# tensorflow/compression

Hardware: AMD Instinct MI355X
Metric: Mpixels/s encode+decode round-trip (bit-exact) (higher is better)
Workload: dtype int32

## Files before the change

compression_amd/_lib.py:

```python
from __future__ import annotations

import ctypes as C
import os

_HERE = os.path.dirname(os.path.abspath(__file__))
LIB_PATH = os.path.join(_HERE, "libtfc_hip.so")

_vp = C.c_void_p
_i64 = C.c_int64
_int = C.c_int

SIGNATURES = {
    "tfc_abi_version": (_int, []),
    "tfc_last_error": (C.c_char_p, []),
    "tfc_profile_enable": (None, [_int]),
    "tfc_set_default_mode": (_int, [_int]),
    "tfc_get_default_mode": (_int, []),
    "tfc_set_chip_shared": (_int, [_int]),
    "tfc_image_to_unit": (_int, [_vp, _vp, _int, C.c_int64, _vp]),
    "tfc_unit_to_image": (_int, [_vp, _int, _vp, C.c_int64, _vp]),
    "tfc_index_prepare": (_int, [_vp, _int, _vp, C.c_int64, _int, _vp]),
    "tfc_build_tables": (_int, [_vp, C.c_int64, C.c_int64, _vp, _vp, C.c_int64, _int, _vp, _vp]),
    "tfc_build_tables_overflow": (_int, [_vp, C.c_int64, C.c_int64, _vp, _vp, C.c_int64, _int, _vp, _vp, _vp]),
    "tfc_deep_factorized_tails": (_int, [_vp, C.c_int64, C.c_int64, _int, _int, _vp, _int, _vp, _vp, _vp]),
    "tfc_pad2d": (_int, [_vp, _vp, _int, C.c_int64, C.c_int64, C.c_int64, C.c_int64, _int, _int, _int, _int, _int, _vp]),
    "tfc_cache_bytes": (_int, [C.POINTER(C.c_longlong)]),
    "tfc_cache_trim": (_int, [C.POINTER(C.c_longlong)]),
    "tfc_encoder_capacity": (_int, [_vp, C.POINTER(_i64)]),
    "tfc_profile_query": (_int, [C.c_char_p, C.POINTER(C.c_double), C.POINTER(_i64)]),
    "tfc_pipe_counters": (_int, [C.POINTER(_i64), C.POINTER(_i64)]),
    "tfc_set_pipe_format": (_int, [_int, _int]),
    "tfc_tables_create": (_int, [_vp, _int, _i64, _i64, _vp, C.POINTER(_vp)]),
    "tfc_tables_count": (_i64, [_vp]),
    "tfc_tables_destroy": (None, [_vp]),
    "tfc_encoder_create": (_int, [_vp, _i64, _vp, C.POINTER(_vp)]),
    "tfc_encoder_create_many": (_int, [_vp, _i64, _int, _vp, _vp]),
    "tfc_encoder_set_mode": (_int, [_vp, _int]),
    "tfc_encoder_set_deferred_errors": (_int, [_vp, _int]),
    "tfc_encoder_encode": (_int, [_vp, _vp, _vp, _i64, _vp]),
    "tfc_encoder_encode_many": (_int, [_int, _vp, _vp, _vp, _i64, _vp]),
    "tfc_encoder_encode_quantized": (_int, [_vp, _vp, _int, _vp, _vp, _i64, _i64, _vp]),
    "tfc_encoder_encode_quantized_indexed": (_int, [_vp, _vp, _int, _vp, _vp, _i64, _vp]),
    "tfc_encoder_encode_quantized_many": (_int, [_int, _vp, _vp, _int, _vp, _vp, _i64, _i64, _vp]),
    "tfc_decoder_decode_dequantized_many": (_int, [_int, _vp, _vp, _int, _vp, _vp, _i64, _i64, _vp]),
    "tfc_encoder_encode_quantized_indexed_many": (_int, [_int, _vp, _vp, _int, _vp, _vp, _i64, _vp]),
    "tfc_decoder_decode_dequantized_indexed_many": (_int, [_int, _vp, _vp, _vp, _int, _vp, _i64, _vp]),
    "tfc_encoder_finalize": (_int, [_vp, _vp, C.POINTER(_i64)]),
    "tfc_encoder_finalize_device": (_int, [_vp, _vp]),
    "tfc_encoder_finalize_device_many": (_int, [_int, _vp, _vp]),
    "tfc_encoder_status": (_int, [_vp, _vp, C.POINTER(_i64)]),
    "tfc_encoder_result": (_int, [_vp, C.POINTER(_vp), C.POINTER(_vp)]),
    "tfc_encoder_read": (_int, [_vp, _vp, _vp, _int, _vp]),
    "tfc_encoder_destroy": (None, [_vp]),
    "tfc_decoder_create": (_int, [_vp, _vp, _vp, _i64, _int, _vp, C.POINTER(_vp)]),
    "tfc_decoder_create_many": (_int, [_vp, _int, _vp, _vp, _vp]),
    "tfc_decoder_set_mode": (_int, [_vp, _int]),
    "tfc_decoder_decode": (_int, [_vp, _vp, _vp, _i64, _vp]),
    "tfc_decoder_decode_many": (_int, [_int, _vp, _vp, _vp, _i64, _vp]),
    "tfc_decoder_decode_dequantized": (_int, [_vp, _vp, _vp, _int, _vp, _vp, _i64, _i64, _vp]),
    "tfc_decoder_finalize": (_int, [_vp, _vp, _vp]),
    "tfc_decoder_finalize_device": (_int, [_vp, _vp, _vp]),
    "tfc_decoder_finalize_device_many": (_int, [_int, _vp, _vp, _vp]),
    "tfc_decoder_status": (_int, [_vp, _vp]),
    "tfc_decoder_destroy": (None, [_vp]),
    "tfc_range_encode": (_int, [_vp, _vp, _int, _vp, _vp, _int, _int, _int, _vp,
                                C.POINTER(_vp), C.POINTER(_i64)]),
    "tfc_range_decode": (_int, [_vp, _i64, _vp, _int, _vp, _vp, _int, _int, _int, _vp, _vp]),
    "tfc_unbounded_index_range_encode": (_int, [_vp, _vp, _i64, _vp, _i64, _i64, _vp, _vp, _int, _int, _int,
                                                _vp, C.POINTER(_vp), C.POINTER(_i64)]),
    "tfc_unbounded_index_range_decode": (_int, [_vp, _i64, _vp, _i64, _vp, _i64, _i64, _vp, _vp, _int, _int,
                                                _int, _vp, _vp]),
    "tfc_stochastic_round": (_int, [_vp, _int, _i64, C.c_float, _vp, _i64, _vp, _vp]),
    "tfc_free": (None, [_vp]),
    "tfc_run_length_workspace": (_i64, [_i64, _i64]),
    "tfc_run_length_encode_size": (_int, [_vp, _int, _i64, _i64, _int, _int, _int, _vp, _vp, C.POINTER(_i64), _vp]),
    "tfc_run_length_encode_write": (_int, [_vp, _int, _i64, _i64, _int, _int, _int, _vp, _vp, _vp, _vp]),
    "tfc_run_length_decode": (_int, [_vp, _vp, _vp, _i64, _i64, _int, _int, _int, _int, _vp, _vp, _vp]),
    "tfc_pmf_to_quantized_cdf": (_int, [_vp, _i64, _i64, _int, _vp, _vp]),
    "tfc_gdn_forward": (_int, [_vp, _vp, _int, _i64, _i64, _vp, _vp, _int, _int, _int, _int, _vp]),
    "tfc_gdn_params_create": (_int, [_vp, _vp, _i64, _int, _vp, C.POINTER(_vp)]),
    "tfc_gdn_params_destroy": (None, [_vp]),
    "tfc_gdn_forward_prepared": (_int, [_vp, _vp, _vp, _i64, _int, _int, _int, _int, _vp]),
    "tfc_gdn_forward_general": (_int, [_vp, _vp, _int, _i64, _i64, _vp, _vp, _int, _int, C.c_float, C.c_float, _vp]),
# ... 138 lines not shown
```

compression_amd/csrc/range_coder.hip:

```cpp
#include <hip/hip_bf16.h>
#include <hip/hip_fp16.h>
#include <hip/hip_runtime.h>

#include <algorithm>
#include <atomic>
#include <cstdlib>
#include <cstring>
#include <type_traits>
#include <memory>
#include <mutex>
#include <string>
#include <vector>

#include "../../include/tfc_hip.h"
#include "common.h"
#include "range_coder_device.h"
#include "range_tables.h"
#include "range_wave.h"

using namespace tfc;


namespace tfc {

// ... 1288 lines not shown
  if (n <= 0) return 0;
  bool batch = n <= kMaxFinalizeJobs;
  for (int k = 0; k < n; ++k) es[k]->touch(st);
  for (int k = 0; k < n && batch; ++k) {
    const tfc_encoder* e = es[k];
    if (e->finalized || e->family != kLanes || e->chunks.size() != 1 || e->streams != es[0]->streams ||
        e->streams == 0 || e->chunks[0].stride != es[0]->chunks[0].stride)
      batch = false;
  }
  if (!batch) {
    for (int k = 0; k < n; ++k)
      if (tfc_encoder_finalize_device(es[k], stream)) return 1;
    return 0;
  }
  const int64_t streams = es[0]->streams;
  FinalizeJobs f;
  f.streams = streams;
  f.n = n;
  const size_t cap = es[0]->chunks[0].data_bytes + 4 * static_cast<size_t>(streams) + 64;
  f.length_off = static_cast<long long>((sizeof(Tail) * streams + 15) & ~size_t{15});
  f.offsets_off = f.length_off + static_cast<long long>(sizeof(long long)) * streams;
  f.blob_off = (f.offsets_off + static_cast<long long>(sizeof(long long)) * (streams + 1) + 15) & ~15ll;
  f.job_bytes = (f.blob_off + static_cast<long long>(cap) + 255) & ~255ll;
  auto group = std::make_shared<DevBuf>();
  TFC_HIP(group->alloc(static_cast<size_t>(f.job_bytes) * n, st));
  f.base = group->as<uint8_t>();
  for (int k = 0; k < n; ++k) {
    EncChunk& c = es[k]->chunks[0];
    f.job[k].state = es[k]->state.as<uint4>();
    f.job[k].chunk = ChunkRef{c.data.as<uint8_t>(), c.off.as<long long>(), c.len_p, c.stride};
  }
  hipLaunchKernelGGL(enc_tail_many_kernel, dim3(static_cast<unsigned>(ceil_div(streams, 256)), static_cast<unsigned>(n)),
                     dim3(256), 0, st, f);
  hipLaunchKernelGGL(scan_lengths_many_kernel, dim3(static_cast<unsigned>(n)), dim3(1024), 0, st, f);
  hipLaunchKernelGGL(enc_pack_many_kernel,
                     dim3(static_cast<unsigned>(ceil_div(streams, kWavesPerBlock)), static_cast<unsigned>(n)),
                     dim3(kBlock), 0, st, f);
  TFC_HIP(hipGetLastError());
  for (int k = 0; k < n; ++k) {
    tfc_encoder* e = es[k];
    e->result_group = group;
    e->offsets.p = f.base + k * f.job_bytes + f.offsets_off;
    e->blob.p = f.base + k * f.job_bytes + f.blob_off;
    e->blob_capacity = static_cast<int64_t>(cap);
    e->chunks.clear();
    e->finalized = true;
  }
  return 0;
}

extern "C" int tfc_debug_pipe_clocks(unsigned long long* out8) {
  TFC_HIP(hipDeviceSynchronize());
  TFC_HIP(hipMemcpyFromSymbol(out8, HIP_SYMBOL(tfc::g_pipe_clock), 8 * sizeof(unsigned long long)));
  return 0;
}
extern "C" int tfc_debug_enc_clocks(unsigned long long* out4) {
  TFC_HIP(hipDeviceSynchronize());
  TFC_HIP(hipMemcpyFromSymbol(out4, HIP_SYMBOL(tfc::g_enc_clock), 4 * sizeof(unsigned long long)));
  return 0;
}

extern "C" int tfc_pipe_counters(int64_t* launches, int64_t* fallback_blocks) {
  if (launches) *launches = pipe_launches().load();
  if (fallback_blocks) {
    unsigned long long v = 0;
    TFC_HIP(hipDeviceSynchronize());
    TFC_HIP(hipMemcpyFromSymbol(&v, HIP_SYMBOL(tfc::g_pipe_fallback_blocks), sizeof(v)));
    *fallback_blocks = static_cast<int64_t>(v);
  }
  return 0;
}

extern "C" int tfc_set_pipe_format(int format, int waves_per_workgroup) {
  if (format < 0 || format > 2 || waves_per_workgroup < 0 || waves_per_workgroup > 8) {
    tfc::fail("tfc_set_pipe_format: format 0 ... 2, waves per workgroup 0 ... 8");
    return -1;
  }
  pipe_waves_value().store(waves_per_workgroup);
  return pipe_format_value().exchange(format);
}

extern "C" int tfc_encoder_set_mode(tfc_encoder* e, int mode) {
  if (mode != TFC_MODE_AUTO && mode != TFC_MODE_LATENCY && mode != TFC_MODE_THROUGHPUT)
    return fail("unknown mode %d", mode);
  if (e->family >= 0) return fail("the mode of a handle is fixed by its first coding call");
  e->mode = mode;
  return 0;
}

extern "C" int tfc_encoder_set_deferred_errors(tfc_encoder* e, int on) {
  e->deferred = on != 0;
  return 0;
}

extern "C" int tfc_encoder_encode(tfc_encoder* e, const int32_t* value, const int32_t* index,
                                  int64_t elems, void* stream) {
  const SymInt32 src{value};
  return encode_jobs(&e, 1, &src, &index, elems, static_cast<hipStream_t>(stream), "tfc_encoder_encode");
}

extern "C" int tfc_encoder_encode_many(int n, tfc_encoder* const* es, const int32_t* const* values,
                                       const int32_t* const* indexes, int64_t elems, void* stream) {
  if (n <= 0) return 0;
  std::vector<SymInt32> srcs(n);
  for (int k = 0; k < n; ++k) srcs[k] = SymInt32{values[k]};
  return encode_jobs(es, n, srcs.data(), indexes, elems, static_cast<hipStream_t>(stream), "tfc_encoder_encode_many");
// ... 720 lines not shown
```

compression_amd/csrc/range_lanes.h:

```cpp
#pragma once

namespace tfc {

__device__ unsigned long long g_pipe_fallback_blocks;
__device__ unsigned long long g_pipe_clock[8];
__device__ unsigned long long g_enc_clock[4];

struct LaneArgs {
  const uint32_t* image;
  int bytes;
  int ntab;
  int precision;
  unsigned int cap;
  int lds_image;
  int lds_wave;
  int defer;
  const unsigned int* guard;
};

__device__ inline unsigned int lds_u16(const unsigned char* lds, unsigned int off) {
  return *reinterpret_cast<const unsigned short*>(lds + off);
}

__device__ inline unsigned int scale16(unsigned int s1, unsigned int c) {
  unsigned int add = c;
  asm volatile("" : "+v"(add));
  return static_cast<unsigned int>((static_cast<unsigned long long>(s1) * c + add) >> 16);
}

constexpr int kLaneJobArgBytes = 3584;
template <typename Src>
struct EncLaneJob {
  Src src;
  const int32_t* index;
  uint4* state;
  uint8_t* chunk;
  unsigned int* chunk_len;
  unsigned long long* first_error;
  unsigned int* overflow_flag;
};
template <typename Src>
struct EncLaneJobs {
  int64_t streams, elems;
  int blocks_per_job, n;
  static constexpr int kMax = kLaneJobArgBytes / sizeof(EncLaneJob<Src>) < 64 ? kLaneJobArgBytes / sizeof(EncLaneJob<Src>) : 64;
  EncLaneJob<Src> job[kMax];
};
template <typename Dst>
struct DecLaneJob {
  Dst dst;
  const int32_t* index;
  const uint8_t* blob;
  const long long* off;
  uint4* state;
  unsigned long long* first_error;
};
template <typename Dst>
struct DecLaneJobs {
// ... 18 lines not shown
  lanes_u32x4 v = {lo.x, lo.y, hi.x, hi.y};
  reinterpret_cast<TFC_AS1 LanePacked<lanes_u32x4>*>((TFC_AS1 void*)p)->v = v;
}
template <typename T>
__device__ inline void lanes_gstore_elem(T* p, const T& v) {
  if (sizeof(T) == 2) {
    unsigned short bits;
    __builtin_memcpy(&bits, &v, 2);
    reinterpret_cast<TFC_AS1 LanePacked<unsigned short>*>((TFC_AS1 void*)p)->v = bits;
  } else {
    unsigned int bits;
    __builtin_memcpy(&bits, &v, 4);
    reinterpret_cast<TFC_AS1 LanePacked<unsigned int>*>((TFC_AS1 void*)p)->v = bits;
  }
}

__device__ inline void lanes_load_image(unsigned char* lds, const LaneArgs& a) {
  const uint4* src = reinterpret_cast<const uint4*>(a.image);
  uint4* dst = reinterpret_cast<uint4*>(lds);
  const int n = (a.bytes + 15) / 16, step = static_cast<int>(blockDim.x);
  int i = threadIdx.x;
  for (; i + 7 * step < n; i += 8 * step) {
    uint4 v[8];
#pragma unroll
    for (int u = 0; u < 8; ++u) v[u] = lanes_gload16(src + i + u * step);
#pragma unroll
    for (int u = 0; u < 8; ++u) dst[i + u * step] = v[u];
  }
  for (; i < n; i += step) dst[i] = src[i];
  __syncthreads();
}

__device__ inline void lanes_pin(unsigned int& a, unsigned int& b, unsigned int& c, unsigned int& d) {
  asm volatile("" : "+v"(a), "+v"(b), "+v"(c), "+v"(d));
}


template <int WORDS>
struct LaneWindow {
  unsigned char* lds;
  const unsigned char* g;
  unsigned int len;
  unsigned int base;
  unsigned int pbase;
  uint2 pend[WORDS];

  __device__ __noinline__ unsigned int tail_word(unsigned int q0) const {
    unsigned int word = 0u;
#pragma nounroll
    for (unsigned int k = 0; k < 4u; ++k)
      if (q0 + k < len) word |= static_cast<unsigned int>(lanes_gload8(g + q0 + k)) << (8u * k);
    return word;
  }
  __device__ void request(unsigned int pos) {
    pbase = pos;
    if (pos + 8u * WORDS <= len) {
#pragma unroll
      for (int w = 0; w < WORDS; w += 2) {
#if defined(TFC_PDEC_ABL) && (TFC_PDEC_ABL & 2)
        const uint4 v = w == 0 ? lanes_gload16(g + pos) : make_uint4(pend[0].x, pend[0].y, pend[1].x, pend[1].y);
#else
        const uint4 v = lanes_gload16(g + pos + 8u * w);
#endif
        pend[w] = make_uint2(v.x, v.y);
        pend[w + 1] = make_uint2(v.z, v.w);
      }
    } else {
#pragma unroll
      for (int w = 0; w < WORDS; ++w) {
        pend[w].x = tail_word(pos + 8u * w);
        pend[w].y = tail_word(pos + 8u * w + 4u);
      }
    }
  }
  __device__ void commit() {
#pragma unroll
    for (int w = 0; w < WORDS; ++w) reinterpret_cast<uint2*>(lds)[w] = pend[w];
    base = pbase;
  }
};

__host__ __device__ constexpr int lane_stride(int payload) {
  return ((payload + 7) & ~7) + ((((payload + 7) & ~7) % 16 == 0) ? 8 : 0);
}


constexpr unsigned int kEncDigitBytes = 32;

template <typename Raw>
struct EncWaveLds {
  static constexpr int kValueWords = 2 * kEncCadence * sizeof(Raw) / 8;
  static constexpr int kIndexWords = 2 * kEncCadence * 4 / 8;
  static constexpr int kDigitStride = lane_stride(kEncDigitBytes + 8);
  static constexpr int kValueStride = lane_stride(8 * kValueWords);
  static constexpr int kIndexStride = lane_stride(8 * kIndexWords);
  static constexpr int kDigits = 0;
  static constexpr int kValue = kDigits + 64 * kDigitStride;
  static constexpr int kIndex = kValue + 64 * kValueStride;
  static constexpr int kBytes = kIndex + 64 * kIndexStride;
};

#define TFC_LENC_A(VAL, R0, R1, LO, HI, NEXTROW, NP)                                        \
  NEXTROW                                                                                 \
  "v_and_b32 v171, 0x7fffffff, v" #R1 "\n\t"                                              \
  "v_cmp_ge_u32 " NP(VAL)                                                                 \
  "v_min_u32 v172, v" #VAL ", v171\n\t"                                                   \
  "v_lshl_add_u32 v172, v172, 1, v" #R0 "\n\t"                                            \
  "ds_read_u16 v" #LO ", v172 offset:2\n\t"                                               \
  "ds_read_u16 v" #HI ", v172 offset:4\n\t"
#define TFC_LENC_B(LO, LOH, HI, HIH, PRE)                                                 \
  PRE                                                                                     \
  "v_mad_u64_u32 v[160:161], s[52:53], v" #LO ", %[S], v[" #LO ":" #LOH "]\n\t"             \
  "v_mad_u64_u32 v[162:163], s[52:53], v" #HI ", %[S], v[" #HI ":" #HIH "]\n\t"             \
  "v_alignbit_b32 v160, v161, v160, 16\n\t"                                               \
  "v_alignbit_b32 v162, v163, v162, 16\n\t"                                               \
  "v_add_u32 v162, -1, v162\n\t"                                                          \
  "v_min_u32 v162, v162, %[S]\n\t"                                                        \
  "v_add_co_u32 v164, vcc, %[BASE], v160\n\t"                                             \
  "v_addc_co_u32 v167, vcc, 0, %[H], vcc\n\t"                                             \
  "v_sub_u32 v165, v162, v160\n\t"                                                        \
  "v_sub_u32 v173, v167, %[H]\n\t"                                                        \
  "v_cmp_gt_u32 vcc, %[K64K], v165\n\t"                                                   \
  "v_cndmask_b32 v174, 0, 1, vcc\n\t"                                                     \
  "v_perm_b32 v166, 0, v167, %[PERM]\n\t"                                                 \
  "ds_write_b16 %[NA], v166\n\t"                                                          \
  "v_or_b32 v168, v173, v174\n\t"                                                         \
  "v_and_b32 v168, v168, %[HAD]\n\t"                                                      \
  "v_lshl_add_u32 %[NA], v168, 1, %[NA]\n\t"                                              \
  "v_lshrrev_b32 v169, 16, v164\n\t"                                                      \
  "v_lshlrev_b32 v170, 16, v164\n\t"                                                      \
  "v_lshl_or_b32 v171, v165, 16, %[KFFFF]\n\t"                                            \
  "v_cndmask_b32 %[BASE], v164, v170, vcc\n\t"                                            \
// ... 872 lines not shown
```

compression_amd/csrc/range_pipe.h:

```cpp
#pragma once

#ifndef TFC_PIPE_TIMING
#define TFC_PIPE_TIMING 0
#endif

namespace tfc {

constexpr int kPipeTile = 256;
constexpr int kPipeEscMax = 32;
constexpr unsigned int kPipeBlock = 16;
constexpr unsigned int kPipeNoCall = 0x0001FFFFu;
constexpr unsigned int kPipeAggregate = 1u << 30;
constexpr unsigned int kPipePrefix = 2u << 30;
constexpr unsigned int kPipeRowsMask = (1u << 30) - 1u;

struct PipeEncArgs {
  const uint16_t* fast16;
  const int2* rows_fast;
  int ntab;
  int tab_entries;
  unsigned int* calls;
  unsigned int* status;
  unsigned int* done;
  unsigned int* fallback;
// ... 842 lines not shown
  if (M < 0) return bit ? -M : (M == -31 ? 32 : M - 1);
  return M - 1;
}

struct PipeDecArgs {
  unsigned short* raw;
  unsigned int* posrec;
  unsigned int* kend;
  uint4* state_out;
  const unsigned short* rowaddr;
  unsigned int* fallback;
  unsigned int* progress;
  unsigned int* tile_done;
  unsigned int* started;
  int rows;
  int groups_per_job;
  int groups;
  int concurrent;
  long long poll_ticks;
};
constexpr unsigned int kPipeFinal = 0x80000000u;
#ifndef TFC_PIPE_RELEASE
#define TFC_PIPE_RELEASE 64
#endif
constexpr unsigned int kPipeRelease = TFC_PIPE_RELEASE;
struct PipeDecJob { const uint8_t* blob; const long long* off; const uint4* state; };
struct PipeDecJobs {
  int64_t streams, elems;
  int blocks_per_job, n;
  PipeDecJob job[64];
};

struct PipeRowJobs {
  int64_t per_job;
  int ntab, n;
  struct { const int32_t* index; unsigned long long* first_error; } job[64];
};
__global__ void __launch_bounds__(256) dec_rows_kernel(const PipeRowJobs jobs, unsigned short* rowaddr) {
  const int k = blockIdx.y;
  const int32_t* index = jobs.job[k].index;
  unsigned short* out = rowaddr + static_cast<size_t>(k) * jobs.per_job;
  for (int64_t i = static_cast<int64_t>(blockIdx.x) * 1024 + threadIdx.x, e = min(jobs.per_job, (static_cast<int64_t>(blockIdx.x) + 1) * 1024);
       i < e; i += 256) {
    int t = tfc_gload(index + i);
    if (t < 0 || t >= jobs.ntab) {
      atomicMin(jobs.job[k].first_error, static_cast<unsigned long long>(i));
      t = 0;
    }
    out[i] = static_cast<unsigned short>(16 * t);
  }
}

struct PipeDecLds {
  static constexpr int kWords = 2 * kPipeBlock * 2 / 8 + 2;
  static constexpr int kStride = lane_stride(8 * kWords);
  static constexpr int kCodes = 0;
  static constexpr int kRows = kCodes + 64 * kStride;
  static constexpr int kBytes = kRows + 64 * kStride;
  static constexpr int kStage = kPipeBlock * 128;
};

#ifndef TFC_PDEC_ABL
#define TFC_PDEC_ABL 0
#endif
#if TFC_PDEC_ABL & 1
#define TFC_PDEC_STORE(KOFF)
#define TFC_PDEC_WAIT2 "s_waitcnt lgkmcnt(1)\n\t"
#else
#define TFC_PDEC_STORE(KOFF) "ds_write_b16 %[STG], v117 offset:" #KOFF "\n\t"
#define TFC_PDEC_WAIT2 "s_waitcnt lgkmcnt(2)\n\t"
#endif
#ifndef TFC_PDEC_PAD
#define TFC_PDEC_PAD 0
#endif
#define TFC_PDEC_PAD2 "v_mov_b32 v139, v139\n\tv_mov_b32 v139, v139\n\t"
#if TFC_PDEC_PAD == 1
#define TFC_PDEC_PAD_A TFC_PDEC_PAD2
#elif TFC_PDEC_PAD == 5
#define TFC_PDEC_PAD_A "s_waitcnt lgkmcnt(15)\n\ts_waitcnt lgkmcnt(15)\n\t"
#else
#define TFC_PDEC_PAD_A
#endif
#if TFC_PDEC_PAD == 2
#define TFC_PDEC_PAD_B TFC_PDEC_PAD2
#else
#define TFC_PDEC_PAD_B
#endif
#if TFC_PDEC_PAD == 3
#define TFC_PDEC_PAD_C TFC_PDEC_PAD2
#else
#define TFC_PDEC_PAD_C
#endif
#if TFC_PDEC_PAD == 4
#define TFC_PDEC_PAD_D TFC_PDEC_PAD2
#else
#define TFC_PDEC_PAD_D
#endif
#define TFC_PDEC_STEP(KOFF, MI, MO, AHEAD, NEXT, PWSTEP)                                    \
  "v_cvt_f32_u32 v111, %[S]\n\t"                                                          \
  "v_add_f32 v111, 1.0, v111\n\t"                                                         \
  "v_rcp_f32 v111, v111\n\t"                                                              \
  TFC_PDEC_PAD_A                                                                          \
  "v_cvt_f32_u32 v110, %[D]\n\t"                                                          \
  "v_fma_f32 v110, -v110, %[SCALE], -%[HSCALE]\n\t"                                       \
  "v_fma_f32 v110, v110, v111, -1.0\n\t"                                                  \
  "v_cvt_i32_f32 v110, v110\n\t"                                                          \
  "v_ashrrev_i32 v111, 6, v110\n\t"                                                       \
// ... 307 lines not shown
            if (D < A) sym = sym > 0u ? sym - 1u : 0u;
            else sym = sym + 1u < nsym ? sym + 1u : nsym - 1u;
            lo = lds_u16(lanes_lds, R.x + 2u * sym + 2u);
            hi = lds_u16(lanes_lds, R.x + 2u * sym + 4u);
            A = scale16(s1, lo);
            b = scale16(s1, hi) - 1u;
            b = hi == 0u ? s1 : b;
          }
        }
        D -= A;
        s1 = b - A;
        const bool ren = (s1 >> 16) == 0u;
        D = ren ? (D << 16) | dig : D;
        s1 = ren ? (s1 << 16) | 0xFFFFu : s1;
        cp += ren ? 2u : 0u;
        entry = pipe_raw_entry(sym, 0);
        M = ((R.y >> 15) & 1u) != 0u && sym == (R.y & 0x7FFFu) ? -1 : 0;
        }
      } else {
        const unsigned int half = scale16(s1, 32768u);
        const unsigned int bit = D >= half ? 1u : 0u;
        const unsigned int A = bit ? half : 0u;
        const unsigned int b = bit ? s1 : half - 1u;
        D -= A;
        s1 = b - A;
        const bool ren = (s1 >> 16) == 0u;
        D = ren ? (D << 16) | dig : D;
        s1 = ren ? (s1 << 16) | 0xFFFFu : s1;
        cp += ren ? 2u : 0u;
        entry = PAIRS ? 0x8001u + bit : pipe_raw_entry(bit, M);
        if (M < 0) {
          if (bit) M = -M;
          else M = M == -31 ? 32 : M - 1;
        } else {
          --M;
        }
      }
      if (M == 0) {
        ++pos;
        pw += INDEXED ? 2u : 16u;
        if (!INDEXED && pw == dir_end) pw = 0u;
        load_row();
      } else {
        R = bin;
      }
      if (to_stage) *reinterpret_cast<unsigned short*>(lanes_lds + stg + 128u * (row - k)) = static_cast<unsigned short>(entry);
      else raw[static_cast<size_t>(row) * 64 + lane] = static_cast<unsigned short>(entry);
    }
  };

#if TFC_PIPE_TIMING
  unsigned long long t_asm = 0ull, n_asm = 0ull, t_commit = 0ull, t_rest = 0ull;
#endif
  auto memory_phase = [&]() __attribute__((always_inline)) {
#if TFC_PIPE_TIMING
    const unsigned long long tm0 = clock64();
#endif
    const unsigned int cpos = cw.base + (cp - cw_off);
    cw.commit();
    cp = cw_off + (cpos - cw.base);
    if (INDEXED) {
      iw.commit();
      pw = iw_off + (2u * pos - iw.base);
    }
#if TFC_PIPE_TIMING
    asm volatile("s_waitcnt lgkmcnt(0)" ::: "memory");
    const unsigned long long tm1 = clock64();
    t_commit += tm1 - tm0;
#endif
    flush();
    if (k != 0u && (k / kPipeBlock) % kPipeRelease == 0u) {
      posrec[static_cast<size_t>(k / kPipeBlock) * 64] = pos + (M != 0 ? 1u : 0u);
      __builtin_amdgcn_fence(__ATOMIC_RELEASE, "agent");
      if (lane == 0u) __hip_atomic_store(&pa.progress[gi], k, __ATOMIC_RELAXED, __HIP_MEMORY_SCOPE_AGENT);
    }
    cw.request(cpos);
    if (INDEXED) iw.request(2u * pos);
    posrec[static_cast<size_t>(k / kPipeBlock) * 64] = pos + (M != 0 ? 1u : 0u);
#if TFC_PIPE_TIMING
    t_rest += clock64() - tm1;
#endif
  };
  auto fast_block = [&](unsigned int& flag) __attribute__((always_inline)) {
#define TFC_PDEC_OPERANDS                                                                                              \
        : [D] "+v"(D), [S] "+v"(s1), [CP] "+v"(cp), [M] "+v"(M), [PW] "+v"(pw), [FLAG] "+v"(flag),                    \
          [R0] "+v"(R.x), [R1] "+v"(R.y), [R2] "+v"(R.z), [R3] "+v"(R.w)                                              \
        : [STG] "v"(stg), [BINROW] "v"(bin_addr_v), [SCALE] "s"(scale), [HSCALE] "v"(hscale),        \
          [K64K] "s"(0x10000u), [KFFFF] "s"(0xFFFFu), [PERM] "s"(0x05040001u), [NSH] "s"(pair_nsh) \
        : "vcc", "memory", "s52", "s53", "s54", "s55", "s56", "s57", "s58", "s59", "v104", "v105", "v106", "v107", "v108", "v109", "v110", "v111", "v112", "v113", \
          "v114", "v115", "v116", "v117", "v118", "v119", "v122", "v123", "v124", "v125", "v126", "v127", "v128",      \
          "v129", "v130", "v131", "v132", "v133", "v134", "v135", "v136", "v137", "v138", "v139", "v140", "v141", "v142", "v143", "v144", "v145"
#if TFC_PIPE_TIMING
    const unsigned long long ta = clock64();
#endif
    if constexpr (INDEXED && PAIRS) asm volatile(TFC_PDEC_BLOCK(TFC_PDEC_STEP_PIX) TFC_PDEC_OPERANDS);
    else if constexpr (PAIRS) asm volatile(TFC_PDEC_BLOCK(TFC_PDEC_STEP_PCH) TFC_PDEC_OPERANDS);
    else if constexpr (INDEXED) asm volatile(TFC_PDEC_BLOCK(TFC_PDEC_STEP_IX) TFC_PDEC_OPERANDS);
    else asm volatile(TFC_PDEC_BLOCK(TFC_PDEC_STEP_CH) TFC_PDEC_OPERANDS);
#if TFC_PIPE_TIMING
    t_asm += clock64() - ta;
    ++n_asm;
#endif
  };
  auto fast_step = [&](unsigned int& flag, unsigned int slot) __attribute__((always_inline)) {
    const unsigned int stg_row = stg + 128u * slot;
    {
      const unsigned int stg = stg_row;
      if constexpr (INDEXED && PAIRS) asm volatile(TFC_PDEC_ONE(TFC_PDEC_STEP_PIX) TFC_PDEC_OPERANDS);
      else if constexpr (PAIRS) asm volatile(TFC_PDEC_ONE(TFC_PDEC_STEP_PCH) TFC_PDEC_OPERANDS);
      else if constexpr (INDEXED) asm volatile(TFC_PDEC_ONE(TFC_PDEC_STEP_IX) TFC_PDEC_OPERANDS);
      else asm volatile(TFC_PDEC_ONE(TFC_PDEC_STEP_CH) TFC_PDEC_OPERANDS);
    }
#undef TFC_PDEC_OPERANDS
  };
  bool gave_up = false;
  while (__any(pos < elems)) {
    if (lds0 == 0u && row_loaded && (INDEXED || static_cast<unsigned int>(la.ntab) >= kPipeBlock)) {
      while (__all(!live || (pos + kPipeBlock <= elems && M > -16)) && k + kPipeBlock <= static_cast<unsigned int>(pa.rows)) {
        memory_phase();
        const unsigned int D0 = D, s10 = s1, cp0 = cp, pw0 = pw;
        const int M0 = M;
        const uint4 R0 = R;
        unsigned int flag = 0u;
        fast_block(flag);
        if (__builtin_expect(__any(live && flag != 0u), 0)) {
          D = D0; s1 = s10; cp = cp0; pw = pw0; M = M0; R = R0;
#pragma nounroll
          for (unsigned int i = 0; i < kPipeBlock; ++i) {
            const unsigned int D1 = D, s11 = s1, cp1 = cp, pw1 = pw;
            const int M1 = M;
            const uint4 R1 = R;
            unsigned int f1 = 0u;
            if (live) fast_step(f1, i);
            if (__any(live && f1 != 0u)) {
              D = D1; s1 = s11; cp = cp1; pw = pw1; M = M1; R = R1;
              gstep(live, k + i, true);
            } else {
              pos += (pw - pw1) / (INDEXED ? 2u : 16u);
              if (!INDEXED) pw -= pw >= dir_end ? dir_end : 0u;
            }
          }
          staged = true;
          staged_k = k;
          k += kPipeBlock;
          continue;
        }
        pos += (pw - pw0) / (INDEXED ? 2u : 16u);
        if (!INDEXED) pw -= pw >= dir_end ? dir_end : 0u;
        staged = true;
        staged_k = k;
        k += kPipeBlock;
      }
      if (!__any(pos < elems)) break;
    }
    if (k + kPipeBlock > static_cast<unsigned int>(pa.rows)) {
      gave_up = true;
      break;
    }
    memory_phase();
    if (!row_loaded) {
      if (M == 0) load_row(); else R = bin;
      row_loaded = true;
    }
    const bool whole = pos + kPipeBlock <= elems;
    const bool blocks = __any(whole);
    if (blocks && __any(!whole && pos < elems && M != 0)) {
      if (pos < elems) {
#pragma unroll
        for (unsigned int i = 0; i < kPipeBlock; ++i) raw[static_cast<size_t>(k + i) * 64 + lane] = static_cast<unsigned short>(kPipeSkipRow);
      }
#pragma nounroll
      for (unsigned int i = 0; i < kPipeBlock; ++i) gstep(!whole && pos < elems && M != 0, k + i);
      k += kPipeBlock;
      continue;
    }
    const bool busy = blocks ? whole : pos < elems;
    const bool sitting = blocks && !whole && pos < elems;
    if (__builtin_expect(lds0 == 0u && blocks && !__any(busy && M <= -16), 1)) {
      if (__any(sitting)) {
        if (sitting) {
#pragma unroll
          for (unsigned int i = 0; i < kPipeBlock; ++i) *reinterpret_cast<unsigned short*>(lanes_lds + stg + 128u * i) = static_cast<unsigned short>(kPipeSkipRow);
        }
      }
      const unsigned int D0 = D, s10 = s1, cp0 = cp, pw0 = pw;
      const int M0 = M;
      const uint4 R0 = R;
      unsigned int flag = 0u;
      if (busy) {
        fast_block(flag);
      }
      if (__builtin_expect(!__any(flag != 0u), 1)) {
        if (busy) {
          pos += (pw - pw0) / (INDEXED ? 2u : 16u);
        }
        if (!INDEXED)
          while (__any(busy && pw >= dir_end)) pw -= pw >= dir_end ? dir_end : 0u;
        staged = true;
        staged_k = k;
        k += kPipeBlock;
        continue;
      }
      D = D0; s1 = s10; cp = cp0; pw = pw0; M = M0; R = R0;
    }
    if (sitting) {
#pragma unroll
      for (unsigned int i = 0; i < kPipeBlock; ++i) raw[static_cast<size_t>(k + i) * 64 + lane] = static_cast<unsigned short>(kPipeSkipRow);
    }
#pragma nounroll
    for (unsigned int i = 0; i < kPipeBlock; ++i) gstep(busy && pos < elems, k + i);
    k += kPipeBlock;
  }
  flush();
  posrec[static_cast<size_t>(k / kPipeBlock) * 64] = pos;
  if (gave_up) {
    if (lane == 0) {
      atomicOr(&pa.fallback[job], 1u);
      __hip_atomic_store(&pa.progress[gi], kPipeFinal, __ATOMIC_RELEASE, __HIP_MEMORY_SCOPE_AGENT);
    }
    return;
  }
  if (lane == 0) pa.kend[gi] = k;
  __builtin_amdgcn_fence(__ATOMIC_RELEASE, "agent");
  if (lane == 0) __hip_atomic_store(&pa.progress[gi], k | kPipeFinal, __ATOMIC_RELAXED, __HIP_MEMORY_SCOPE_AGENT);
  if (gi == 0 && lane == 0) {
    g_pipe_clock[2] = clock64() - clk0;
    g_pipe_clock[3] = wall_clock64() - wall0;
#if TFC_PIPE_TIMING
    g_pipe_clock[5] = t_asm | (t_commit << 32);
    g_pipe_clock[7] = n_asm | (static_cast<unsigned long long>(k) << 16) | (t_rest << 32);
#endif
  }
  if (live) {
    const unsigned int cpos = cw.base + (cp - cw_off);
    const unsigned char* srcp = J.blob + o0;
    unsigned int window = 0u;
    for (int i = -4; i < 0; ++i) {
      const long long q = static_cast<long long>(cpos) + i;
      window = (window << 8) | ((q >= 0 && q < static_cast<long long>(len)) ? srcp[q] : 0u);
    }
    pa.state_out[static_cast<size_t>(gi) * 64 + lane] = make_uint4(window - D, s1, window, cpos >> 1);
  }
}

constexpr int kParseRows = 128;
constexpr unsigned int kParseMargin = 96;

constexpr int kParseEscTables = 2048;

struct PipePairMap { const int* adjust; };
template <bool INDEXED, bool PAIRS, typename Dst>
__global__ void __launch_bounds__(256) dec_parse_kernel(const DecLaneJobs<Dst> jobs, const PipeDecArgs pa, const DecRow* dir, int ntab,
                                                        const PipePairMap pm) {
  constexpr int kPitch = 66;
  __shared__ unsigned short buf[kParseRows * kPitch];
  __shared__ unsigned int escsym[kParseEscTables];
  __shared__ unsigned int incomplete;
  const unsigned int tiles = static_cast<unsigned int>(pa.rows) / kParseRows + 1u;
  const unsigned int gi = blockIdx.x % static_cast<unsigned int>(pa.groups), kt = blockIdx.x / static_cast<unsigned int>(pa.groups);
  const unsigned int job = gi / static_cast<unsigned int>(pa.groups_per_job);
  const unsigned int wv = gi % static_cast<unsigned int>(pa.groups_per_job);
  const DecLaneJob<Dst>& J = jobs.job[job];
  const unsigned int tid = threadIdx.x, lane = tid & 63u;
  const unsigned int k0 = kt * kParseRows;
  unsigned int* const tile_done = pa.tile_done + static_cast<size_t>(gi) * tiles + kt;
  unsigned int kend;
  bool final = true;
  if (pa.concurrent) {
    const unsigned int need = k0 + kParseRows + kParseMargin;
    unsigned int* const abandon = pa.started + 1;
    unsigned int v = 0u;
    if (tid == 0u) {
      unsigned int seen = ~0u, go = 1u;
      long long t0 = 0;
      if (__hip_atomic_load(abandon, __ATOMIC_RELAXED, __HIP_MEMORY_SCOPE_AGENT) != 0u) go = 0u;
      while (go) {
        v = __hip_atomic_load(&pa.progress[gi], __ATOMIC_RELAXED, __HIP_MEMORY_SCOPE_AGENT);
        if ((v & kPipeFinal) || v >= need) break;
        const long long now = static_cast<long long>(wall_clock64());
        if (v != seen) { seen = v; t0 = now; }
// ... 115 lines not shown
```

include/tfc_hip.h:

```cpp
#ifndef TFC_HIP_H_
#define TFC_HIP_H_

#include <stdint.h>

#ifdef __cplusplus
extern "C" {
#endif

typedef struct tfc_tables tfc_tables;
typedef struct tfc_encoder tfc_encoder;
typedef struct tfc_decoder tfc_decoder;

#define TFC_ABI_VERSION 2
int tfc_abi_version(void);
const char* tfc_last_error(void);

void tfc_profile_enable(int on);
int tfc_profile_query(const char* kernel, double* total_ms, int64_t* launches);
int tfc_pipe_counters(int64_t* launches, int64_t* fallback_blocks);
int tfc_set_pipe_format(int format, int waves_per_workgroup);

#define TFC_MODE_AUTO 0
#define TFC_MODE_LATENCY 1
#define TFC_MODE_THROUGHPUT 2
int tfc_set_default_mode(int mode);
int tfc_get_default_mode(void);

int tfc_set_chip_shared(int shared);
int tfc_image_to_unit(const void* x, void* y, int dtype, int64_t n, void* stream);
int tfc_unit_to_image(const void* x, int dtype, void* y, int64_t n, void* stream);
int tfc_index_prepare(const void* indexes, int dtype, int32_t* out, int64_t n, int num_tables, void* stream);
int tfc_pad2d(const void* x, void* y, int elem_bytes, int64_t n, int64_t h, int64_t w, int64_t c, int top, int bottom,
              int left, int right, int reflect, void* stream);
int tfc_cache_bytes(long long* bytes);
int tfc_cache_trim(long long* released);


int tfc_tables_create(const int32_t* lookup, int rank, int64_t rows, int64_t cols,
                      void* stream, tfc_tables** out);
int64_t tfc_tables_count(const tfc_tables* t);
void tfc_tables_destroy(tfc_tables* t);


int tfc_encoder_create(const tfc_tables* tables, int64_t streams, void* stream,
                       tfc_encoder** out);

int tfc_encoder_create_many(const tfc_tables* tables, int64_t streams, int n, void* stream,
                            tfc_encoder** out);

int tfc_encoder_set_mode(tfc_encoder* e, int mode);
int tfc_encoder_set_deferred_errors(tfc_encoder* e, int on);

int tfc_encoder_encode(tfc_encoder* e, const int32_t* value, const int32_t* index,
                       int64_t elems, void* stream);

int tfc_encoder_encode_many(int n, tfc_encoder* const* e, const int32_t* const* value,
                            const int32_t* const* index, int64_t elems, void* stream);

int tfc_encoder_encode_quantized(tfc_encoder* e, const void* y, int dtype,
                                 const float* qoffset, const int32_t* cdf_offset,
                                 int64_t channels, int64_t elems, void* stream);

int tfc_encoder_encode_quantized_indexed(tfc_encoder* e, const void* y, int dtype,
                                         const int32_t* index, const int32_t* cdf_offset,
                                         int64_t elems, void* stream);

int tfc_encoder_encode_quantized_many(int n, tfc_encoder* const* e, const void* const* y, int dtype,
                                      const float* qoffset, const int32_t* cdf_offset,
                                      int64_t channels, int64_t elems, void* stream);
int tfc_encoder_encode_quantized_indexed_many(int n, tfc_encoder* const* e, const void* const* y, int dtype,
                                              const int32_t* const* index, const int32_t* cdf_offset,
                                              int64_t elems, void* stream);
// ... 315 lines not shown
```

Before: 62010.

## Skip LDS window refills in pipelined decoder when current window still suffices

The pipelined range decoder now grows its per-lane LDS code/row windows and, each block, checks wave-wide whether the current window still covers the bytes needed for the next block. The refill is issued only when needed, and its commit is moved after the block so the global load overlaps decode work. This is meant to cut redundant global loads and LDS writes per block. In exchange it adds register pressure from explicit refill buffers, a larger LDS footprint, and new debug counters plus an export function.

```diff
diff --git a/compression_amd/_lib.py b/compression_amd/_lib.py
--- a/compression_amd/_lib.py
+++ b/compression_amd/_lib.py
@@ -29,6 +29,7 @@
     "tfc_encoder_capacity": (_int, [_vp, C.POINTER(_i64)]),
     "tfc_profile_query": (_int, [C.c_char_p, C.POINTER(C.c_double), C.POINTER(_i64)]),
     "tfc_pipe_counters": (_int, [C.POINTER(_i64), C.POINTER(_i64)]),
+    "tfc_debug_pipe_window": (_int, [C.POINTER(_i64), C.POINTER(_i64), C.POINTER(_i64)]),
     "tfc_set_pipe_format": (_int, [_int, _int]),
     "tfc_tables_create": (_int, [_vp, _int, _i64, _i64, _vp, C.POINTER(_vp)]),
     "tfc_tables_count": (_i64, [_vp]),
diff --git a/compression_amd/csrc/range_coder.hip b/compression_amd/csrc/range_coder.hip
--- a/compression_amd/csrc/range_coder.hip
+++ b/compression_amd/csrc/range_coder.hip
@@ -1364,6 +1364,15 @@
 extern "C" int tfc_debug_pipe_clocks(unsigned long long* out8) {
   TFC_HIP(hipDeviceSynchronize());
   TFC_HIP(hipMemcpyFromSymbol(out8, HIP_SYMBOL(tfc::g_pipe_clock), 8 * sizeof(unsigned long long)));
+  return 0;
+}
+extern "C" int tfc_debug_pipe_window(int64_t* phases, int64_t* refills, int64_t* index_refills) {
+  unsigned long long v[3] = {0, 0, 0};
+  TFC_HIP(hipDeviceSynchronize());
+  TFC_HIP(hipMemcpyFromSymbol(v, HIP_SYMBOL(tfc::g_pipe_window), sizeof(v)));
+  if (phases) *phases = static_cast<int64_t>(v[0]);
+  if (refills) *refills = static_cast<int64_t>(v[1]);
+  if (index_refills) *index_refills = static_cast<int64_t>(v[2]);
   return 0;
 }
 extern "C" int tfc_debug_enc_clocks(unsigned long long* out4) {
diff --git a/compression_amd/csrc/range_lanes.h b/compression_amd/csrc/range_lanes.h
--- a/compression_amd/csrc/range_lanes.h
+++ b/compression_amd/csrc/range_lanes.h
@@ -4,6 +4,7 @@
 
 __device__ unsigned long long g_pipe_fallback_blocks;
 __device__ unsigned long long g_pipe_clock[8];
+__device__ unsigned long long g_pipe_window[3];
 __device__ unsigned long long g_enc_clock[4];
 
 struct LaneArgs {
@@ -128,32 +129,36 @@
       if (q0 + k < len) word |= static_cast<unsigned int>(lanes_gload8(g + q0 + k)) << (8u * k);
     return word;
   }
-  __device__ void request(unsigned int pos) {
-    pbase = pos;
+  __device__ void request(unsigned int pos, uint2 (&words)[WORDS]) const {
     if (pos + 8u * WORDS <= len) {
 #pragma unroll
       for (int w = 0; w < WORDS; w += 2) {
 #if defined(TFC_PDEC_ABL) && (TFC_PDEC_ABL & 2)
-        const uint4 v = w == 0 ? lanes_gload16(g + pos) : make_uint4(pend[0].x, pend[0].y, pend[1].x, pend[1].y);
+        const uint4 v = w == 0 ? lanes_gload16(g + pos) : make_uint4(words[0].x, words[0].y, words[1].x, words[1].y);
 #else
         const uint4 v = lanes_gload16(g + pos + 8u * w);
 #endif
-        pend[w] = make_uint2(v.x, v.y);
-        pend[w + 1] = make_uint2(v.z, v.w);
+        words[w] = make_uint2(v.x, v.y);
+        words[w + 1] = make_uint2(v.z, v.w);
       }
     } else {
 #pragma unroll
       for (int w = 0; w < WORDS; ++w) {
-        pend[w].x = tail_word(pos + 8u * w);
-        pend[w].y = tail_word(pos + 8u * w + 4u);
-      }
-    }
-  }
-  __device__ void commit() {
+        words[w].x = tail_word(pos + 8u * w);
+        words[w].y = tail_word(pos + 8u * w + 4u);
+      }
+    }
+  }
+  __device__ void commit(unsigned int pos, const uint2 (&words)[WORDS]) {
 #pragma unroll
-    for (int w = 0; w < WORDS; ++w) reinterpret_cast<uint2*>(lds)[w] = pend[w];
-    base = pbase;
-  }
+    for (int w = 0; w < WORDS; ++w) reinterpret_cast<uint2*>(lds)[w] = words[w];
+    base = pos;
+  }
+  __device__ void request(unsigned int pos) {
+    pbase = pos;
+    request(pos, pend);
+  }
+  __device__ void commit() { commit(pbase, pend); }
 };
 
 __host__ __device__ constexpr int lane_stride(int payload) {
diff --git a/compression_amd/csrc/range_pipe.h b/compression_amd/csrc/range_pipe.h
--- a/compression_amd/csrc/range_pipe.h
+++ b/compression_amd/csrc/range_pipe.h
@@ -918,7 +918,7 @@
 }
 
 struct PipeDecLds {
-  static constexpr int kWords = 2 * kPipeBlock * 2 / 8 + 2;
+  static constexpr int kWords = 2 * kPipeBlock * 2 / 8 + 4;
   static constexpr int kStride = lane_stride(8 * kWords);
   static constexpr int kCodes = 0;
   static constexpr int kRows = kCodes + 64 * kStride;
@@ -1332,21 +1332,35 @@
 #if TFC_PIPE_TIMING
   unsigned long long t_asm = 0ull, n_asm = 0ull, t_commit = 0ull, t_rest = 0ull;
 #endif
-  auto memory_phase = [&]() __attribute__((always_inline)) {
+  static_assert(8 * L::kWords >= 4 * kPipeBlock + 2, "a window holds two blocks and the entry read ahead");
+  constexpr unsigned int kWindowNeed = 4u * kPipeBlock + 2u;
+  struct WindowRefill {
+    uint2 code[L::kWords], rows[L::kWords];
+    unsigned int code_pos, rows_pos;
+    bool code_pending, rows_pending;
+  };
+  unsigned int n_phase = 0u, n_refill = 0u, n_irefill = 0u;
+  auto park = [&](const WindowRefill& rq) __attribute__((always_inline)) {
 #if TFC_PIPE_TIMING
     const unsigned long long tm0 = clock64();
 #endif
-    const unsigned int cpos = cw.base + (cp - cw_off);
-    cw.commit();
-    cp = cw_off + (cpos - cw.base);
-    if (INDEXED) {
-      iw.commit();
+    if (rq.code_pending) {
+      const unsigned int cpos = cw.base + (cp - cw_off);
+      cw.commit(rq.code_pos, rq.code);
+      cp = cw_off + (cpos - cw.base);
+    }
+    if (INDEXED && rq.rows_pending) {
+      iw.commit(rq.rows_pos, rq.rows);
       pw = iw_off + (2u * pos - iw.base);
     }
 #if TFC_PIPE_TIMING
     asm volatile("s_waitcnt lgkmcnt(0)" ::: "memory");
+    t_commit += clock64() - tm0;
+#endif
+  };
+  auto phase_decide = [&](WindowRefill& rq) __attribute__((always_inline)) {
+#if TFC_PIPE_TIMING
     const unsigned long long tm1 = clock64();
-    t_commit += tm1 - tm0;
 #endif
     flush();
     if (k != 0u && (k / kPipeBlock) % kPipeRelease == 0u) {
@@ -1354,12 +1368,43 @@
       __builtin_amdgcn_fence(__ATOMIC_RELEASE, "agent");
       if (lane == 0u) __hip_atomic_store(&pa.progress[gi], k, __ATOMIC_RELAXED, __HIP_MEMORY_SCOPE_AGENT);
     }
-    cw.request(cpos);
-    if (INDEXED) iw.request(2u * pos);
     posrec[static_cast<size_t>(k / kPipeBlock) * 64] = pos + (M != 0 ? 1u : 0u);
+    ++n_phase;
+    rq.code_pos = cw.base + (cp - cw_off);
+    rq.code_pending = !__all((cp - cw_off) + kWindowNeed <= 8u * L::kWords);
+    rq.rows_pos = 2u * pos;
+    rq.rows_pending = INDEXED && !__all((rq.rows_pos - iw.base) + kWindowNeed <= 8u * L::kWords);
+    n_refill += rq.code_pending ? 1u : 0u;
+    n_irefill += rq.rows_pending ? 1u : 0u;
 #if TFC_PIPE_TIMING
     t_rest += clock64() - tm1;
 #endif
+  };
+  auto phase_request = [&](WindowRefill& rq) __attribute__((always_inline)) {
+#if TFC_PIPE_TIMING
+    const unsigned long long tm1 = clock64();
+#endif
+    if (rq.code_pending) {
+      cw.request(rq.code_pos, rq.code);
+    } else {
+#pragma unroll
+      for (int w = 0; w < L::kWords; ++w) asm("" : "=v"(rq.code[w].x), "=v"(rq.code[w].y));
+    }
+    if (INDEXED) {
+      if (rq.rows_pending) {
+        iw.request(rq.rows_pos, rq.rows);
+      } else {
+#pragma unroll
+        for (int w = 0; w < L::kWords; ++w) asm("" : "=v"(rq.rows[w].x), "=v"(rq.rows[w].y));
+      }
+    }
+#if TFC_PIPE_TIMING
+    t_rest += clock64() - tm1;
+#endif
+  };
+  auto memory_phase = [&](WindowRefill& rq) __attribute__((always_inline)) {
+    phase_decide(rq);
+    phase_request(rq);
   };
   auto fast_block = [&](unsigned int& flag) __attribute__((always_inline)) {
 #define TFC_PDEC_OPERANDS                                                                                              \
@@ -1393,43 +1438,52 @@
     }
 #undef TFC_PDEC_OPERANDS
   };
+  cw.commit();
+  if (INDEXED) iw.commit();
   bool gave_up = false;
   while (__any(pos < elems)) {
     if (lds0 == 0u && row_loaded && (INDEXED || static_cast<unsigned int>(la.ntab) >= kPipeBlock)) {
       while (__all(!live || (pos + kPipeBlock <= elems && M > -16)) && k + kPipeBlock <= static_cast<unsigned int>(pa.rows)) {
-        memory_phase();
-        const unsigned int D0 = D, s10 = s1, cp0 = cp, pw0 = pw;
-        const int M0 = M;
-        const uint4 R0 = R;
-        unsigned int flag = 0u;
-        fast_block(flag);
-        if (__builtin_expect(__any(live && flag != 0u), 0)) {
-          D = D0; s1 = s10; cp = cp0; pw = pw0; M = M0; R = R0;
-#pragma nounroll
-          for (unsigned int i = 0; i < kPipeBlock; ++i) {
-            const unsigned int D1 = D, s11 = s1, cp1 = cp, pw1 = pw;
-            const int M1 = M;
-            const uint4 R1 = R;
-            unsigned int f1 = 0u;
-            if (live) fast_step(f1, i);
-            if (__any(live && f1 != 0u)) {
-              D = D1; s1 = s11; cp = cp1; pw = pw1; M = M1; R = R1;
-              gstep(live, k + i, true);
-            } else {
-              pos += (pw - pw1) / (INDEXED ? 2u : 16u);
-              if (!INDEXED) pw -= pw >= dir_end ? dir_end : 0u;
+        WindowRefill rq;
+        phase_decide(rq);
+        auto block = [&]() __attribute__((always_inline)) {
+          const unsigned int D0 = D, s10 = s1, cp0 = cp, pw0 = pw;
+          const int M0 = M;
+          const uint4 R0 = R;
+          unsigned int flag = 0u;
+          fast_block(flag);
+          if (__builtin_expect(__any(live && flag != 0u), 0)) {
+            D = D0; s1 = s10; cp = cp0; pw = pw0; M = M0; R = R0;
+  #pragma nounroll
+            for (unsigned int i = 0; i < kPipeBlock; ++i) {
+              const unsigned int D1 = D, s11 = s1, cp1 = cp, pw1 = pw;
+              const int M1 = M;
+              const uint4 R1 = R;
+              unsigned int f1 = 0u;
+              if (live) fast_step(f1, i);
+              if (__any(live && f1 != 0u)) {
+                D = D1; s1 = s11; cp = cp1; pw = pw1; M = M1; R = R1;
+                gstep(live, k + i, true);
+              } else {
+                pos += (pw - pw1) / (INDEXED ? 2u : 16u);
+                if (!INDEXED) pw -= pw >= dir_end ? dir_end : 0u;
+              }
             }
+          } else {
+            pos += (pw - pw0) / (INDEXED ? 2u : 16u);
+            if (!INDEXED) pw -= pw >= dir_end ? dir_end : 0u;
           }
           staged = true;
           staged_k = k;
           k += kPipeBlock;
-          continue;
+        };
+        if (rq.code_pending || rq.rows_pending) {
+          phase_request(rq);
+          block();
+          park(rq);
+        } else {
+          block();
         }
-        pos += (pw - pw0) / (INDEXED ? 2u : 16u);
-        if (!INDEXED) pw -= pw >= dir_end ? dir_end : 0u;
-        staged = true;
-        staged_k = k;
-        k += kPipeBlock;
       }
       if (!__any(pos < elems)) break;
     }
@@ -1437,7 +1491,8 @@
       gave_up = true;
       break;
     }
-    memory_phase();
+    WindowRefill rq;
+    memory_phase(rq);
     if (!row_loaded) {
       if (M == 0) load_row(); else R = bin;
       row_loaded = true;
@@ -1452,6 +1507,7 @@
 #pragma nounroll
       for (unsigned int i = 0; i < kPipeBlock; ++i) gstep(!whole && pos < elems && M != 0, k + i);
       k += kPipeBlock;
+      park(rq);
       continue;
     }
     const bool busy = blocks ? whole : pos < elems;
@@ -1479,6 +1535,7 @@
         staged = true;
         staged_k = k;
         k += kPipeBlock;
+        park(rq);
         continue;
       }
       D = D0; s1 = s10; cp = cp0; pw = pw0; M = M0; R = R0;
@@ -1490,6 +1547,7 @@
 #pragma nounroll
     for (unsigned int i = 0; i < kPipeBlock; ++i) gstep(busy && pos < elems, k + i);
     k += kPipeBlock;
+    park(rq);
   }
   flush();
   posrec[static_cast<size_t>(k / kPipeBlock) * 64] = pos;
@@ -1506,6 +1564,9 @@
   if (gi == 0 && lane == 0) {
     g_pipe_clock[2] = clock64() - clk0;
     g_pipe_clock[3] = wall_clock64() - wall0;
+    g_pipe_window[0] = n_phase;
+    g_pipe_window[1] = n_refill;
+    g_pipe_window[2] = n_irefill;
 #if TFC_PIPE_TIMING
     g_pipe_clock[5] = t_asm | (t_commit << 32);
     g_pipe_clock[7] = n_asm | (static_cast<unsigned long long>(k) << 16) | (t_rest << 32);
diff --git a/include/tfc_hip.h b/include/tfc_hip.h
--- a/include/tfc_hip.h
+++ b/include/tfc_hip.h
@@ -18,6 +18,7 @@
 void tfc_profile_enable(int on);
 int tfc_profile_query(const char* kernel, double* total_ms, int64_t* launches);
 int tfc_pipe_counters(int64_t* launches, int64_t* fallback_blocks);
+int tfc_debug_pipe_window(int64_t* phases, int64_t* refills, int64_t* index_refills);
 int tfc_set_pipe_format(int format, int waves_per_workgroup);
 
 #define TFC_MODE_AUTO 0
```

Result: faster. 63080 (median of 6 runs) (+1.7%).
